# cdcseacave/openMVS

Measured on NVIDIA H100. Metric: Mpix/sec depth+normal (1920x1080, 9 neighbours), higher is better.
Workload: dtype f32

## Files before the change

### openmvs_b200/csrc/capi.cu

```cuda
#include "../../include/b200mvs.h"
#include "pm_common.cuh"
#include "sgm_front_sched.h"
#include <cuda.h>
#include <cmath>
#include <cstdio>
#include <cstring>
#include <string>
#include <vector>
#include <chrono>
#include <algorithm>
#include <cstdlib>

cudaError_t pm_configure_device();
cudaError_t pm_launch_score(const PMParams& P, bool geom, cudaStream_t s);
cudaError_t pm_launch_sweep(const PMParams& P, const void* tmapRef, bool geom, bool fourCtas, cudaStream_t s);
void pm_tma_box(int* w, int* h);
cudaError_t pm_launch_finalize(int n, float keep, const float4* plane, const float* cost, const uint32_t* bestViews,
	float* depth, float* normal, float* conf, uint32_t* viewsMap, cudaStream_t s);
cudaError_t pm_launch_pack(int n, const float* depth, const float* normal, float4* plane, cudaStream_t s);
cudaError_t pm_launch_unpack(int n, const float4* plane, float* depth, float* normal, cudaStream_t s);
struct SGMPixel { unsigned long long idx; short dmin, dmax; int pad; };
struct SGMParams {
	const float* lgray; const uchar3* lbgr; const float* rgray;
	int w, h, vw, vh;
	const SGMPixel* px;
	uint8_t* costs; uint16_t* accums;
	int P1;
	uint16_t P2s[256];
	int maxNumDisp;
};
cudaError_t sgm_configure_device();
cudaError_t sgm_launch_maxdisp(const SGMPixel* px, int n, unsigned long long numCosts, int* out8, cudaStream_t s);
cudaError_t sgm_launch_cost(const SGMParams& P, cudaStream_t s);
cudaError_t sgm_cost_tc_configure();
bool sgm_cost_tc_supports(int num);
cudaError_t sgm_cost_tc_launch(const SGMParams& P, int dmin, int num, cudaStream_t s);
cudaError_t sgm_launch_aggregate(const SGMParams& P, int dir, bool store, cudaStream_t s);
cudaError_t sgm_launch_aggregate_uniform(const SGMParams& P, int dir, int dmin, int num, bool ring, cudaStream_t s);
cudaError_t sgm_front_launch(const SGMParams& P, const FrontArgs& A, int blocks, int pd, cudaStream_t s);
int sgm_front_blocks_per_sm(int num, int pd);
bool sgm_front_supports(int num);
cudaError_t sgm_launch_wta(const SGMParams& P, int nVol, unsigned long long volStride, const uint16_t* more, int16_t* disparity, uint16_t* cost, cudaStream_t s);
cudaError_t sgm_launch_wta_uniform(const SGMParams& P, const uint16_t* second, int dmin, int num, int16_t* disparity, uint16_t* cost, cudaStream_t s);
int sgm_max_disparities();
cudaError_t sgm_launch_cross_check(int16_t* l2r, const int16_t* r2l, int w, int h, int th, cudaStream_t s);
cudaError_t sgm_launch_refine(const SGMPixel* px, const uint16_t* accums, int16_t* disparity, int n, int steps, cudaStream_t s);
#define FLT_MAX_NBR 16
struct FltView { const float* depth; const float* conf; int w, h; double fx, fy, cx, cy; double R[9], C[3]; };
// ... 224 lines not shown
	}
	return fn;
}

int prepare_ref_tmap(b200mvs_ctx* ctx, const DView& ref, cudaStream_t s) {
	ctx->tmapValid = false;
	EncodeTiledFn enc = ctx->dbg.noTMA ? nullptr : encode_tiled_fn();
	if (!enc) return B200MVS_OK;
	const float* base = ref.img; size_t pitchB = (size_t)ref.pitch*4;
	if (((uintptr_t)base & 15) || (pitchB & 15)) {
		pitchB = (((size_t)ref.w*4)+15)&~(size_t)15;
		CK(ctx->refPad.reserve(pitchB*ref.h));
		CK(cudaMemcpy2DAsync(ctx->refPad.p, pitchB, ref.img, (size_t)ref.pitch*4, (size_t)ref.w*4, ref.h, cudaMemcpyDeviceToDevice, s));
		base = ctx->refPad.as<float>();
	}
	int bw, bh; pm_tma_box(&bw, &bh);
	const cuuint64_t dims[2] = {(cuuint64_t)ref.w, (cuuint64_t)ref.h};
	const cuuint64_t strides[1] = {(cuuint64_t)pitchB};
	const cuuint32_t box[2] = {(cuuint32_t)bw, (cuuint32_t)bh};
	const cuuint32_t estr[2] = {1, 1};
	const CUresult r = enc(&ctx->tmapRef, CU_TENSOR_MAP_DATA_TYPE_FLOAT32, 2, (void*)base, dims, strides, box, estr,
		CU_TENSOR_MAP_INTERLEAVE_NONE, CU_TENSOR_MAP_SWIZZLE_NONE, CU_TENSOR_MAP_L2_PROMOTION_NONE, CU_TENSOR_MAP_FLOAT_OOB_FILL_NONE);
	ctx->tmapValid = (r == CUDA_SUCCESS);
	return B200MVS_OK;
}

int launch_sweep_timed(b200mvs_ctx* ctx, const PMParams& P, bool geom, cudaStream_t s) {
	if (ctx->timeSweeps) {
		while ((int)ctx->sweepEv.size() < 2*(ctx->nSweepEv+1)) {
			cudaEvent_t e; CK(cudaEventCreate(&e)); ctx->sweepEv.push_back(e);
		}
		CK(cudaEventRecord(ctx->sweepEv[2*ctx->nSweepEv], s));
	}
	CK(pm_launch_sweep(P, ctx->tmapValid ? &ctx->tmapRef : nullptr, geom, ctx->dbg.sweepFourCtas != 0, s)); ++ctx->launches;
	if (ctx->timeSweeps) {
		CK(cudaEventRecord(ctx->sweepEv[2*ctx->nSweepEv+1], s));
		++ctx->nSweepEv;
	}
	return B200MVS_OK;
}

int estimate_on_device(b200mvs_ctx* ctx, const DView* views, int nViews, float dMin, float dMax, int nGeometricIter,
	float* d_depth, float* d_normal, float* d_conf, uint32_t* d_views, cudaStream_t s)
{
	const b200mvs_params& o = ctx->prm;
	const int W = views[0].w, H = views[0].h;
	const bool geometric = nGeometricIter >= 0;
	int nSweepsPhoto, nRPhoto, nSweeps, nR;
	engine_schedule(o, false, nSweepsPhoto, nRPhoto);
	engine_schedule(o, geometric, nSweeps, nR);
	const int sweepBase = geometric ? nSweepsPhoto + nGeometricIter*nSweeps : 0;
	const int totalScale = !geometric ? std::max(0, o.nSubResolutionLevels) : 0;
	const size_t P0 = (size_t)W*H;
	if (ctx->mask && (ctx->maskW != W || ctx->maskH != H))
		return fail(ctx, B200MVS_ERR_ARG, "ignore-mask size differs from the reference image");
	CK(ctx->plane.reserve(P0*sizeof(float4)));
	CK(ctx->cost.reserve(P0*sizeof(float)));
	CK(ctx->best.reserve(P0*sizeof(uint32_t)));
	if (totalScale > 0) {
		CK(ctx->prior.reserve(P0*sizeof(float)));
		CK(ctx->lowPlane.reserve((size_t)(W/2+2)*(H/2+2)*sizeof(float4)));
		if (ctx->mask) CK(ctx->maskLevel.reserve((size_t)(W/2+2)*(H/2+2)));
		if ((int)ctx->pyr.size() < nViews) ctx->pyr.resize(nViews);
		for (int i = 0; i < nViews; ++i) {
			const size_t dw = (size_t)cvRoundI(views[i].w*0.5), dh = (size_t)cvRoundI(views[i].h*0.5);
			CK(ctx->pyr[i].reserve(dw*dh*sizeof(float)*(views[i].dmap ? 2 : 1)));
		}
// ... 472 lines not shown
	for (int i = 0; i < nViews; ++i)
		to_dview(views[i], views[i].image, views[i].stride_bytes ? views[i].stride_bytes/4 : views[i].width,
			views[i].depth, views[i].dstride_bytes ? views[i].dstride_bytes/4 : views[i].dwidth, dv[i]);
	{ const int rc2 = prepare_ref_tmap(ctx, dv[0], s); if (rc2) return rc2; }
	build_params(ctx->prm, dv.data(), nViews, dMin, dMax, lowres, (float4*)plane4, cost, nullptr, P, geom);
	P.tma = ctx->tmapValid ? 1 : 0;
	return B200MVS_OK;
}
int b200mvs_pm_score(b200mvs_ctx* ctx, const b200mvs_view* views, int nViews, float dMin, float dMax,
	const float* lowres, float* plane4, float* cost, void* stream)
{
	PMParams P; bool geom;
	if (!ctx) return B200MVS_ERR_ARG;
	CK(cudaSetDevice(ctx->device));
	cudaStream_t s = stream ? (cudaStream_t)stream : ctx->stream;
	int rc = block_params(ctx, views, nViews, dMin, dMax, lowres, plane4, cost, s, P, geom);
	if (rc) return rc;
	CK(pm_launch_score(P, geom, s));
	return B200MVS_OK;
}
int b200mvs_pm_sweep(b200mvs_ctx* ctx, const b200mvs_view* views, int nViews, float dMin, float dMax,
	const float* lowres, int sweep, int half, int nRandomIters, float* plane4, float* cost, void* stream)
{
	PMParams P; bool geom;
	if (!ctx) return B200MVS_ERR_ARG;
	CK(cudaSetDevice(ctx->device));
	cudaStream_t s = stream ? (cudaStream_t)stream : ctx->stream;
	int rc = block_params(ctx, views, nViews, dMin, dMax, lowres, plane4, cost, s, P, geom);
	if (rc) return rc;
	P.sweep = sweep; P.nRandomIters = nRandomIters;
	for (int colour = 0; colour < 2; ++colour) {
		if (half >= 0 && half != colour) continue;
		P.colour = colour;
		CK(pm_launch_sweep(P, ctx->tmapValid ? &ctx->tmapRef : nullptr, geom, ctx->dbg.sweepFourCtas != 0, s));
	}
	return B200MVS_OK;
}
int b200mvs_pm_finalize(b200mvs_ctx* ctx, int width, int height, float keep, const float* plane4, const float* cost,
	float* depth, float* normal, float* conf, void* stream)
{
	if (!ctx || !plane4 || !cost || !depth || !normal || !conf) return B200MVS_ERR_ARG;
	CK(cudaSetDevice(ctx->device));
	CK(pm_launch_finalize(width*height, keep, (const float4*)plane4, cost, nullptr, depth, normal, conf, nullptr,
		stream ? (cudaStream_t)stream : ctx->stream));
	return B200MVS_OK;
}

void b200mvs_sgm_default_params(b200mvs_sgm_params* p) { p->P1 = 3; p->P2 = 4; p->P2alpha = 14.f; p->P2beta = 38.f; }

int b200mvs_sgm_match_device(b200mvs_ctx* ctx, const float* leftGray, const uint8_t* leftBGR, const float* rightGray,
	int width, int height, const b200mvs_sgm_pixel* pixels, uint64_t numCosts, const b200mvs_sgm_params* prm,
	int stages, uint8_t* costs, uint16_t* accums, int16_t* disparity, uint16_t* cost, void* stream, b200mvs_stats* stats)
{
	if (!ctx) return B200MVS_ERR_ARG;
	if (!leftGray || !leftBGR || !rightGray || !pixels || width <= 6 || height <= 6 || numCosts == 0)
		return fail(ctx, B200MVS_ERR_ARG, "sgm: null image/pixel map or image too small");
	if ((stages & 4) && (!disparity || !cost))
		return fail(ctx, B200MVS_ERR_ARG, "sgm: null output map");
	b200mvs_sgm_params def; b200mvs_sgm_default_params(&def);
	if (!prm) prm = &def;
	CK(cudaSetDevice(ctx->device));
	cudaStream_t s = stream ? (cudaStream_t)stream : ctx->stream;
	static_assert(sizeof(b200mvs_sgm_pixel) == sizeof(SGMPixel), "pixel record layout");
	SGMParams P; memset(&P, 0, sizeof(P));
	P.lgray = leftGray; P.lbgr = (const uchar3*)leftBGR; P.rgray = rightGray;
	P.w = width; P.h = height; P.vw = width-6; P.vh = height-6;
	P.px = (const SGMPixel*)pixels;
// ... 446 lines not shown
```

### openmvs_b200/csrc/pm_kernels.cu

```cuda
#include "pm_common.cuh"
#include <math_constants.h>
#include <cstring>
#include <cuda.h>

namespace {

constexpr int BLOCK_X = 32;
constexpr int BLOCK_Y = 8;

constexpr int NTHREADS = BLOCK_X*BLOCK_Y;

struct PatchW {
	float2* s;
	float sumW, normSq0;
	__device__ __forceinline__ void set(int k, float a, float b) { s[k*NTHREADS] = make_float2(a, b); }
	__device__ __forceinline__ float2 get(int k) const { return s[k*NTHREADS]; }
};

constexpr int TILE_W = 2*BLOCK_X+2*PM_HALF;
constexpr int TILE_H = BLOCK_Y+2*PM_HALF;
constexpr int TILE_BYTES = TILE_W*TILE_H*4;

__device__ __forceinline__ uint32_t smem_u32(const void* p) { return (uint32_t)__cvta_generic_to_shared(p); }
__device__ __forceinline__ void mbar_init(uint64_t* bar, unsigned count) {
	asm volatile("mbarrier.init.shared::cta.b64 [%0], %1;" :: "r"(smem_u32(bar)), "r"(count) : "memory");
}
__device__ __forceinline__ void mbar_expect_tx(uint64_t* bar, unsigned bytes) {
	asm volatile("mbarrier.arrive.expect_tx.shared::cta.b64 _, [%0], %1;" :: "r"(smem_u32(bar)), "r"(bytes) : "memory");
}
__device__ __forceinline__ void mbar_wait(uint64_t* bar, unsigned parity) {
	asm volatile(
		"{\n"
		".reg .pred p;\n"
		"WAIT_LOOP:\n"
		"mbarrier.try_wait.parity.shared::cta.b64 p, [%0], %1;\n"
		"@p bra WAIT_DONE;\n"
		"bra WAIT_LOOP;\n"
		"WAIT_DONE:\n"
		"}\n" :: "r"(smem_u32(bar)), "r"(parity) : "memory");
}
__device__ __forceinline__ void tma_load_2d(void* dst, const CUtensorMap* map, int c0, int c1, uint64_t* bar) {
	asm volatile("cp.async.bulk.tensor.2d.shared::cluster.global.mbarrier::complete_tx::bytes [%0], [%1, {%2, %3}], [%4];"
		:: "r"(smem_u32(dst)), "l"(map), "r"(c0), "r"(c1), "r"(smem_u32(bar)) : "memory");
}

__device__ __forceinline__ void fill_patch_tile(const float* __restrict__ tile, int lx, int ly, PatchW& p) {
	const float sigmaColor = -1.f/(2.f*0.1f*0.1f);
	const float sigmaSpatial = -1.f/(2.f*9.f);
	const float center = tile[ly*TILE_W + lx];
	float acc = 0.f, sumW = 0.f;
	float w[PM_TEXELS], I[PM_TEXELS];
	#pragma unroll
	for (int i = 0; i < 5; ++i) {
		#pragma unroll
		for (int j = 0; j < 5; ++j) {
			const int dy = 2*i-PM_HALF, dx = 2*j-PM_HALF;
			const float v = tile[(ly+dy)*TILE_W + (lx+dx)];
			const float dI = v-center;
			const float wgt = expf(dI*dI*sigmaColor + float(dx*dx+dy*dy)*sigmaSpatial);
			w[i*5+j] = wgt;
			I[i*5+j] = v;
			acc += v*wgt;
			sumW += wgt;
		}
	}
	const float tm = acc/sumW;
	float nsq = 0.f;
	#pragma unroll
	for (int k = 0; k < PM_TEXELS; ++k) {
		const float t = I[k]-tm;
		const float tw = w[k]*t;
		nsq += tw*t;
		p.set(k, w[k], tw);
	}
	p.sumW = sumW;
	p.normSq0 = nsq;
}

__device__ __forceinline__ void fill_patch(const float* __restrict__ img, int pitch, int x, int y, PatchW& p) {
	const float sigmaColor = -1.f/(2.f*0.1f*0.1f);
	const float sigmaSpatial = -1.f/(2.f*9.f);
	const float center = __ldg(img + (size_t)y*pitch + x);
	float acc = 0.f, sumW = 0.f;
	float w[PM_TEXELS], I[PM_TEXELS];
	#pragma unroll
	for (int i = 0; i < 5; ++i) {
		#pragma unroll
		for (int j = 0; j < 5; ++j) {
			const int dy = 2*i-PM_HALF, dx = 2*j-PM_HALF;
			const float v = __ldg(img + (size_t)(y+dy)*pitch + (x+dx));
			const float dI = v-center;
			const float wgt = expf(dI*dI*sigmaColor + float(dx*dx+dy*dy)*sigmaSpatial);
			w[i*5+j] = wgt;
			I[i*5+j] = v;
			acc += v*wgt;
			sumW += wgt;
		}
	}
	const float tm = acc/sumW;
	float nsq = 0.f;
	#pragma unroll
	for (int k = 0; k < PM_TEXELS; ++k) {
		const float t = I[k]-tm;
		const float tw = w[k]*t;
		nsq += tw*t;
		p.set(k, w[k], tw);
	}
	p.sumW = sumW;
	p.normSq0 = nsq;
}

struct Hyp {
	float d;
	float3 n;
	float invd;
	float3 ms;
	float smooth;
};

struct Close {
	float d[4];
	float3 n[4];
	float rx[4], ry[4];
	unsigned mask;
};

__device__ __forceinline__ float fast_rcp(float x) { float r; asm("rcp.approx.ftz.f32 %0, %1;" : "=f"(r) : "f"(x)); return r; }
__device__ __forceinline__ float pow2neg(unsigned i) { return __int_as_float((int)(127u-i)<<23); }
__device__ __forceinline__ float dot3(const float3& a, const float3& b) { return a.x*b.x + a.y*b.y + a.z*b.z; }

__device__ __forceinline__ bool sample_depth_masked(const float* __restrict__ img, int pitch, float px, float py, float ref, float& v) {
	const int lx = (int)px, ly = (int)py;
	const float x = px-lx, x1 = 1.f-x, y = py-ly, y1 = 1.f-y;
	const float* r0 = img + (size_t)ly*pitch + lx;
	const float x0y0 = __ldg(r0), x1y0 = __ldg(r0+1), x0y1 = __ldg(r0+pitch), x1y1 = __ldg(r0+pitch+1);
	const bool b00 = fabsf(ref-x0y0)/ref < 0.03f, b10 = fabsf(ref-x1y0)/ref < 0.03f;
	const bool b01 = fabsf(ref-x0y1)/ref < 0.03f, b11 = fabsf(ref-x1y1)/ref < 0.03f;
	if (!b00 && !b10 && !b01 && !b11)
		return false;
	v = y1*(x1*(b00 ? x0y0 : (b10 ? x1y0 : (b01 ? x0y1 : x1y1))) + x*(b10 ? x1y0 : (b00 ? x0y0 : (b11 ? x1y1 : x0y1)))) +
	    y *(x1*(b01 ? x0y1 : (b11 ? x1y1 : (b00 ? x0y0 : x1y0))) + x*(b11 ? x1y1 : (b01 ? x0y1 : (b10 ? x1y0 : x0y0))));
	return true;
}

__device__ __forceinline__ void fetch_texels(const void* __restrict__ tex, int pitch, int lx, int ly,
	float& v00, float& v10, float& v01, float& v11)
{
	unsigned long long addr;
	const unsigned idx = (unsigned)(ly*pitch + lx);
	asm("mad.wide.u32 %0, %1, %2, %3;" : "=l"(addr) : "r"(idx), "r"(4u), "l"((unsigned long long)tex));
	const float* r0 = (const float*)addr;
	const float* r1 = r0+pitch;
	asm("ld.global.nc.L1::evict_last.f32 %0, [%1];" : "=f"(v00) : "l"(r0));
	asm("ld.global.nc.L1::evict_last.f32 %0, [%1+4];" : "=f"(v10) : "l"(r0));
	asm("ld.global.nc.L1::evict_last.f32 %0, [%1];" : "=f"(v01) : "l"(r1));
	asm("ld.global.nc.L1::evict_last.f32 %0, [%1+4];" : "=f"(v11) : "l"(r1));
}

template <bool GEOM>
__device__ __forceinline__ float score_view(const PMParams& P, const PMView& V, const PatchW& pt,
	float fx, float fy, float X0x, float X0y, const Hyp& h, float priorF, float priorD)
{
	float c0x = fmaf(V.Hm[0], h.ms.x, V.A[0]), c0y = fmaf(V.Hm[1], h.ms.x, V.A[3]), c0z = fmaf(V.Hm[2], h.ms.x, V.A[6]);
	float c1x = fmaf(V.Hm[0], h.ms.y, V.A[1]), c1y = fmaf(V.Hm[1], h.ms.y, V.A[4]), c1z = fmaf(V.Hm[2], h.ms.y, V.A[7]);
	const float xc = fmaf(V.Hm[0], h.invd, fmaf(V.A[0], fx, fmaf(V.A[1], fy, V.A[2])));
	const float yc = fmaf(V.Hm[1], h.invd, fmaf(V.A[3], fx, fmaf(V.A[4], fy, V.A[5])));
	const float zc = fmaf(V.Hm[2], h.invd, fmaf(V.A[6], fx, fmaf(V.A[7], fy, V.A[8])));
	float bx = fmaf(-4.f, c0x+c1x, xc), by = fmaf(-4.f, c0y+c1y, yc), bz = fmaf(-4.f, c0z+c1z, zc);
	c0x *= 2.f; c0y *= 2.f; c0z *= 2.f; c1x *= 2.f; c1y *= 2.f; c1z *= 2.f;
	const float xmax = float(V.w-2), ymax = float(V.h-2);
	bool ok;
	{
		const float x1 = fmaf(4.f, c0x, bx), y1 = fmaf(4.f, c0y, by), z1 = fmaf(4.f, c0z, bz);
		const float x2 = fmaf(4.f, c1x, bx), y2 = fmaf(4.f, c1y, by), z2 = fmaf(4.f, c1z, bz);
		const float x3 = fmaf(4.f, c1x, x1), y3 = fmaf(4.f, c1y, y1), z3 = fmaf(4.f, c1z, z1);
		const float zmin = fminf(fminf(bz, z1), fminf(z2, z3)), zmax = fmaxf(fmaxf(bz, z1), fmaxf(z2, z3));
		const float i0 = fast_rcp(bz), i1 = fast_rcp(z1), i2 = fast_rcp(z2), i3 = fast_rcp(z3);
		const float pxmin = fminf(fminf(bx*i0, x1*i1), fminf(x2*i2, x3*i3)), pxmax = fmaxf(fmaxf(bx*i0, x1*i1), fmaxf(x2*i2, x3*i3));
		const float pymin = fminf(fminf(by*i0, y1*i1), fminf(y2*i2, y3*i3)), pymax = fmaxf(fmaxf(by*i0, y1*i1), fmaxf(y2*i2, y3*i3));
		ok = (zmin > 0.f || zmax < 0.f) && pxmin >= 1.f && pymin >= 1.f && pxmax <= xmax && pymax <= ymax;
		ok = ok && (bx*i0 == bx*i0) && (x1*i1 == x1*i1) && (x2*i2 == x2*i2) && (x3*i3 == x3*i3)
		        && (by*i0 == by*i0) && (y1*i1 == y1*i1) && (y2*i2 == y2*i2) && (y3*i3 == y3*i3);
	}
	if (!__any_sync(__activemask(), ok))
		return P.thRobust;
	if (!ok) { bx = by = bz = 1.f; c0x = c0y = c0z = c1x = c1y = c1z = 0.f; }
	const void* tex = V.img;
	int pitch = V.pitch;
	asm volatile("" : "+r"(pitch), "+l"(tex));
	float sum = 0.f, sumSq = 0.f, num = 0.f;
	#pragma unroll
	for (int i = 0; i < 5; ++i) {
		float X = bx, Y = by, Z = bz;
		#pragma unroll
		for (int j = 0; j < 5; ++j) {
			const float iz = fast_rcp(Z);
			const float px = X*iz, py = Y*iz;
			const int lx = __float2int_rz(px), ly = __float2int_rz(py);
			const float ax = px-(float)lx, ay = py-(float)ly;
			float v00, v10, v01, v11;
			fetch_texels(tex, pitch, lx, ly, v00, v10, v01, v11);
			const float top = fmaf(ax, v10-v00, v00), bot = fmaf(ax, v11-v01, v01);
			const float v = fmaf(ay, bot-top, top);
			const float2 wk = pt.get(i*5+j);
			const float vw = v*wk.x;
			sum += vw; sumSq = fmaf(v, vw, sumSq); num = fmaf(v, wk.y, num);
			X += c0x; Y += c0y; Z += c0z;
		}
		bx += c1x; by += c1y; bz += c1z;
	}
	const bool bad = !ok;
	if (bad)
		return P.thRobust;
	const float normSq1 = sumSq - sum*sum/pt.sumW;
	const float nrmSq = pt.normSq0*normSq1;
	if (nrmSq <= 1e-16f)
		return P.thRobust;
	const float ncc = fminf(fmaxf(num/sqrtf(nrmSq), -1.f), 1.f);
	float score = (1.f-ncc)*h.smooth;
	if (GEOM) {
		if (V.dmap) {
			float consistency = 4.f;
			const float Xx = X0x*h.d, Xy = X0y*h.d, Xz = h.d;
			const float X1x = V.Tl[0]*Xx + V.Tl[1]*Xy + V.Tl[2]*Xz + V.Tm[0];
			const float X1y = V.Tl[3]*Xx + V.Tl[4]*Xy + V.Tl[5]*Xz + V.Tm[1];
			const float X1z = V.Tl[6]*Xx + V.Tl[7]*Xy + V.Tl[8]*Xz + V.Tm[2];
			if (X1z > 0.f) {
				const float x1x = X1x/X1z, x1y = X1y/X1z;
				if (x1x >= 1.f && x1y >= 1.f && x1x <= float(V.dw-2) && x1y <= float(V.dh-2)) {
					float depth1;
					if (sample_depth_masked(V.dmap, V.dpitch, x1x, x1y, X1z, depth1)) {
						const float Px = x1x*depth1, Py = x1y*depth1, Pz = depth1;
						const float Bx = V.Tr[0]*Px + V.Tr[1]*Py + V.Tr[2]*Pz + V.Tn[0];
						const float By = V.Tr[3]*Px + V.Tr[4]*Py + V.Tr[5]*Pz + V.Tn[1];
// ... 4 lines not shown
					}
				}
			}
			score += P.geomWeight*consistency;
		}
	}
	if (priorD > 0.f) {
		const float deltaDepth = fminf(fabsf(priorD-h.d)/priorD, 0.5f);
		score = (1.f-priorF)*score + priorF*deltaDepth;
	}
	return fminf(2.f, score);
}

template <bool GEOM>
__device__ __forceinline__ float score_pixel(const PMParams& P, const PatchW& pt,
	float fx, float fy, float X0x, float X0y, const Hyp& h, float priorF, float priorD, uint32_t& best)
{
	float s0 = CUDART_INF_F, s1 = CUDART_INF_F;
	int i0 = 255, i1 = 255;
	#pragma unroll 1
	for (int v = 0; v < P.nViews; ++v) {
		const float s = score_view<GEOM>(P, P.views[v], pt, fx, fy, X0x, X0y, h, priorF, priorD);
		if (s < s0) { s1 = s0; i1 = i0; s0 = s; i0 = v; }
		else if (s < s1) { s1 = s; i1 = v; }
	}
	if (P.nViews <= 1 || s1 >= P.thRobust) {
		best = 0xFFFFFF00u | (uint32_t)i0;
		return s0;
	}
	best = 0xFFFF0000u | ((uint32_t)i1<<8) | (uint32_t)i0;
	return (s0+s1)*0.5f;
}

__device__ __forceinline__ void make_hyp(const PMParams& P, float X0x, float X0y, float d, const float3& n,
	const Close& cl, bool useClose, Hyp& h)
{
	h.d = d; h.n = n;
	h.invd = 1.f/d;
	const float nX0 = n.x*X0x + n.y*X0y + n.z;
	const float s = 1.f/(nX0*d);
	h.ms = make_float3(n.x*P.ifx*s, (n.x*P.sk + n.y*P.ify)*s, (n.x*P.ox + n.y*P.oy + n.z)*s);
	float smooth = 1.f;
	if (useClose) {
		const float planeD = -d*nX0;
		const float nn = dot3(n, n);
		#pragma unroll
		for (int k = 0; k < 4; ++k) {
			if (cl.mask & (1u<<k)) {
				const float dist = (n.x*cl.rx[k] + n.y*cl.ry[k] + n.z)*cl.d[k] + planeD;
				const float rd = dist/d;
				const float factorDepth = expf(rd*rd*P.smoothSigmaDepth);
				float ca = dot3(n, cl.n[k])/sqrtf(nn*dot3(cl.n[k], cl.n[k]));
				ca = fminf(fmaxf(ca, -1.f), 1.f);
				const float ang = acosf(ca);
				const float factorNormal = expf(ang*ang*P.smoothSigmaNormal);
				smooth *= (1.f-P.smoothBonusDepth*factorDepth)*(1.f-P.smoothBonusNormal*factorNormal);
			}
		}
	}
	h.smooth = smooth;
}

__device__ __forceinline__ float3 dir2normal(float a, float b) {
	float sa, ca, sb, cb;
	sincosf(a, &sa, &ca);
	sincosf(b, &sb, &cb);
	return make_float3(ca*sb, sa*sb, cb);
}
__device__ __forceinline__ float3 random_normal(float u1, float u2, float X0x, float X0y) {
	const float kPI = 3.14159265358979323846f;
	const float a = 0.f + (kPI-0.f)*u1;
	const float b = 0.5f*kPI + (kPI-0.5f*kPI)*u2;
	float3 n = dir2normal(a, b);
	if (n.x*X0x + n.y*X0y + n.z > 0.f)
		n = make_float3(-n.x, -n.y, -n.z);
	return n;
}
__device__ __forceinline__ void correct_normal(float3& n, float X0x, float X0y) {
	const float cosAngLen = n.x*X0x + n.y*X0y + n.z;
	if (cosAngLen >= 0.f) {
		const float kPI = 3.14159265358979323846f;
		const float vlen = sqrtf(X0x*X0x + X0y*X0y + 1.f);
		const float ang = fminf((acosf(cosAngLen/vlen) - 0.5f*kPI)*1.01f, -0.001f);
		float3 w = make_float3(n.y*1.f - n.z*X0y, n.z*X0x - n.x*1.f, n.x*X0y - n.y*X0x);
		const float inv = 1.f/sqrtf(dot3(w, w));
// ... 22 lines not shown
	const bool inside = x >= PM_HALF && y >= PM_HALF && x < P.W-PM_HALF && y < P.H-PM_HALF;
	PatchW pt;
	pt.s = smemW + threadIdx.y*BLOCK_X + threadIdx.x;
	float priorD = 0.f, priorF = 0.f;
	bool ok = inside && !(P.mask && P.mask[(size_t)y*P.maskPitch + x] == 0);
	if (ok) {
		fill_patch(P.img0, P.pitch0, x, y, pt);
		if (P.lowres)
			priorD = fmaxf(__ldg(P.lowres + idx), 0.f);
		if (pt.normSq0 < P.thMagnitudeSq && !(priorD > 0.f))
			ok = false;
	}
	if (!ok) {
		P.plane[idx] = make_float4(0.f, 0.f, 0.f, 0.f);
		P.cost[idx] = 2.f;
		if (P.bestViews) P.bestViews[idx] = 0xFFFFFFFFu;
		return;
	}
	if (priorD > 0.f)
		priorF = expf(pt.normSq0*(-1.f/0.02f));
	const float fx = float(x), fy = float(y);
	const float X0x = fx*P.ifx + fy*P.sk + P.ox, X0y = fy*P.ify + P.oy;
	float4 pl = P.plane[idx];
	float3 n = make_float3(pl.x, pl.y, pl.z);
	float d = pl.w;
	const uint4 r = philox4x32_10(make_uint4((uint32_t)idx, 0u, 0u, 0u), make_uint2(P.seed, 0xB200C0DEu));
	if (!(P.dMin <= d && d < P.dMax)) {
		const float s = P.dMinSqr + (P.dMaxSqr-P.dMinSqr)*u32_to_unit(r.x);
		d = s*s;
		n = random_normal(u32_to_unit(r.y), u32_to_unit(r.z), X0x, X0y);
	} else if (n.x*X0x + n.y*X0y + n.z >= 0.f) {
		n = random_normal(u32_to_unit(r.x), u32_to_unit(r.y), X0x, X0y);
	}
	Close cl; cl.mask = 0;
	Hyp h;
	make_hyp(P, X0x, X0y, d, n, cl, false, h);
	uint32_t best;
	const float c = score_pixel<GEOM>(P, pt, fx, fy, X0x, X0y, h, priorF, priorD, best);
	P.plane[idx] = make_float4(n.x, n.y, n.z, d);
	P.cost[idx] = c;
	if (P.bestViews) P.bestViews[idx] = best;
}

template <bool GEOM, int MINB>
__global__ void __launch_bounds__(BLOCK_X*BLOCK_Y, MINB)
pm_sweep_kernel(const __grid_constant__ PMParams P, const __grid_constant__ CUtensorMap tmapRef)
{
	extern __shared__ __align__(128) unsigned char smemRaw[];
	float2* smemW = (float2*)smemRaw;
	float* tile = (float*)(smemRaw + PM_TEXELS*NTHREADS*sizeof(float2));
	uint64_t* bar = (uint64_t*)(tile + TILE_W*TILE_H);
	const int tid = threadIdx.y*BLOCK_X + threadIdx.x;
	if (P.tma) {
		if (tid == 0) {
			mbar_init(bar, 1);
			asm volatile("fence.proxy.async.shared::cta;" ::: "memory");
		}
		__syncthreads();
		if (tid == 0) {
			mbar_expect_tx(bar, TILE_BYTES);
			tma_load_2d(tile, &tmapRef, (int)blockIdx.x*(2*BLOCK_X)-PM_HALF, (int)blockIdx.y*BLOCK_Y-PM_HALF, bar);
		}
		mbar_wait(bar, 0);
	}
	const int y = blockIdx.y*BLOCK_Y + threadIdx.y;
	const int x = blockIdx.x*(2*BLOCK_X) + 2*threadIdx.x + ((y+P.colour)&1);
	if (x < PM_HALF || y < PM_HALF || x >= P.W-PM_HALF || y >= P.H-PM_HALF)
		return;
	if (P.mask && P.mask[(size_t)y*P.maskPitch + x] == 0)
		return;
	const int W = P.W, H = P.H;
	const size_t idx = (size_t)y*W + x;
	PatchW pt;
	pt.s = smemW + tid;
	if (P.tma)
		fill_patch_tile(tile, 2*(int)threadIdx.x + ((y+P.colour)&1) + PM_HALF, (int)threadIdx.y + PM_HALF, pt);
	else
		fill_patch(P.img0, P.pitch0, x, y, pt);
	float priorD = 0.f, priorF = 0.f;
	if (P.lowres)
		priorD = fmaxf(__ldg(P.lowres + idx), 0.f);
	if (pt.normSq0 < P.thMagnitudeSq && !(priorD > 0.f))
		return;
	if (priorD > 0.f)
		priorF = expf(pt.normSq0*(-1.f/0.02f));
	const float fx = float(x), fy = float(y);
	const float X0x = fx*P.ifx + fy*P.sk + P.ox, X0y = fy*P.ify + P.oy;

	const int dir = P.sweep & 1;
	const int nProp = P.propagation, farRings = P.farRings;
	Close cl; cl.mask = 0;
	unsigned todo = 0;
	unsigned farSel = 0;
	#pragma unroll
	for (int k = 0; k < 4; ++k) {
		const int kk = dir ? (k^2) : k;
		const int ox = (kk == 0) ? -1 : (kk == 2) ? 1 : 0;
		const int oy = (kk == 1) ? -1 : (kk == 3) ? 1 : 0;
		const bool ok = (kk == 0) ? (x > PM_HALF) : (kk == 1) ? (y > PM_HALF) : (kk == 2) ? (x < W-PM_HALF) : (y < H-PM_HALF);
		cl.d[k] = 0.f; cl.n[k] = make_float3(0.f, 0.f, 0.f); cl.rx[k] = 0.f; cl.ry[k] = 0.f;
		if (ok) {
			const size_t nidx = (size_t)(y+oy)*W + (x+ox);
			const float4 np = P.plane[nidx];
			const float nc = P.cost[nidx];
			bool changed = !cost_unchanged(nc);
			float bestC = 3.f;
			if (np.w > 0.f) {
				cl.mask |= 1u<<k;
				cl.d[k] = np.w; cl.n[k] = make_float3(np.x, np.y, np.z);
				const float nfx = float(x+ox), nfy = float(y+oy);
				cl.rx[k] = nfx*P.ifx + nfy*P.sk + P.ox; cl.ry[k] = nfy*P.ify + P.oy;
				bestC = fabsf(nc);
			}
			if (k < nProp) {
				unsigned ring = 0;
				for (int f = 1; f <= farRings; ++f) {
					const int qx = x+ox*(2*f+1), qy = y+oy*(2*f+1);
					if (qx < PM_HALF || qy < PM_HALF || qx >= W-PM_HALF || qy >= H-PM_HALF)
						break;
					const float fc = P.cost[(size_t)qy*W + qx];
					changed = changed || !cost_unchanged(fc);
					if (fabsf(fc) < bestC) { bestC = fabsf(fc); ring = (unsigned)f; }
				}
				if (bestC < P.keep && (changed || !P.skipUnchanged)) {
					todo |= 1u<<k;
					farSel |= ring<<(2*k);
				}
			}
		}
	}
	const float4 pl = P.plane[idx];
	float conf = fabsf(P.cost[idx]);
	float depth = pl.w;
	float3 normal = make_float3(pl.x, pl.y, pl.z);
	uint32_t bestViews = P.bestViews ? P.bestViews[idx] : 0xFFFFFFFFu;

	const int nR = P.nRandomIters;
	const int nRl = P.evalCap > 0 ? min(nR, max(P.evalCap-__popc(todo), 1)) : nR;
	const uint2 key = make_uint2(P.seed, 0xB200C0DEu);
	const uint32_t phase = 1u + (uint32_t)P.sweep;
	int mode = 0;
	bool entered = false;
	bool useClose = true;
	unsigned idxScale = 0;
	float scaleRange = 1.f, depthRange = 0.f, pa = 0.f, pb = 0.f;
	int nRestart = 0, nRefine = 0;
	#pragma unroll 1
	for (;;) {
		bool have = false, isRefine = false, alive = false, uc = true;
		float hd = 0.f, na = 0.f, nb = 0.f; float3 hn = make_float3(0.f, 0.f, 1.f);
		if (todo != 0u) {
			const int k = __ffs((int)todo)-1;
			todo &= todo-1u;
			const int kk = dir ? (k^2) : k;
			const int dist = 2*(int)((farSel>>(2*k))&3u)+1;
			const int qx = x + ((kk == 0) ? -dist : (kk == 2) ? dist : 0);
			const int qy = y + ((kk == 1) ? -dist : (kk == 3) ? dist : 0);
			const float4 qp = P.plane[(size_t)qy*W + qx];
			const bool vertical = (kk & 1) != 0;
			const float ncomp = vertical ? qp.y : qp.x;
			const float nx1 = vertical ? X0y : fmaf(fx, P.ifx, P.ox0);
			const float x1 = vertical ? fmaf(float(qy), P.ify, P.oy) : fmaf(float(qx), P.ifx, P.ox0);
			const float denom = qp.z + nx1*ncomp;
			hd = qp.w;
			if (!(fabsf(denom) < 0.0001f)) {
				const float dn = qp.w*(qp.z + x1*ncomp)/denom;
				if (P.dMin <= dn && dn < P.dMax)
// ... 16 lines not shown
					pa = atan2f(normal.y, normal.x);
					pb = acosf(normal.z);
				}
			}
			if (mode == 1 && nRestart >= nRl) mode = 3;
			alive = (mode == 1) || (mode == 2 && nRefine < nRl);
			uc = useClose;
			if (mode == 1) {
				const uint4 r = philox4x32_10(make_uint4((uint32_t)idx, phase, (uint32_t)nRestart, 0u), key);
				++nRestart;
				const float s = P.dMinSqr + (P.dMaxSqr-P.dMinSqr)*u32_to_unit(r.x);
				hd = s*s;
				hn = random_normal(u32_to_unit(r.y), u32_to_unit(r.z), X0x, X0y);
				have = true;
			} else if (mode == 2 && nRefine < nRl) {
				const uint4 r = philox4x32_10(make_uint4((uint32_t)idx, phase, (uint32_t)(nR+nRefine), 0u), key);
				++nRefine;
				hd = depth + depthRange*scaleRange*(2.f*u32_to_unit(r.x)-1.f);
				if (P.dMin <= hd && hd < P.dMax) {
					na = pa + P.angle1Range*scaleRange*(2.f*u32_to_unit(r.y)-1.f);
					nb = pb + P.angle2Range*scaleRange*(2.f*u32_to_unit(r.z)-1.f);
					hn = dir2normal(na, nb);
					have = hn.x*X0x + hn.y*X0y + hn.z < 0.f;
					isRefine = true;
				}
			}
		}
		if (!__any_sync(__activemask(), alive))
			break;
		if (!__any_sync(__activemask(), have))
			continue;
		if (have) {
			Hyp h;
			make_hyp(P, X0x, X0y, hd, hn, cl, uc, h);
			uint32_t bv;
			const float nconf = score_pixel<GEOM>(P, pt, fx, fy, X0x, X0y, h, priorF, priorD, bv);
			if (conf > nconf) {
				conf = nconf; depth = hd; normal = hn; bestViews = bv;
				if (isRefine) {
					pa = na; pb = nb;
					++idxScale;
					scaleRange = pow2neg(idxScale);
				}
			}
		}
	}
	const bool same = depth == pl.w && normal.x == pl.x && normal.y == pl.y && normal.z == pl.z;
	P.plane[idx] = make_float4(normal.x, normal.y, normal.z, depth);
	P.cost[idx] = (same && P.skipUnchanged) ? -conf : conf;
	if (P.bestViews) P.bestViews[idx] = bestViews;
}

__global__ void pm_finalize_kernel(int n, float keep, const float4* __restrict__ plane, const float* __restrict__ cost,
	const uint32_t* __restrict__ bestViews, float* __restrict__ depth, float* __restrict__ normal, float* __restrict__ conf,
	uint32_t* __restrict__ viewsMap)
{
	const int i = blockIdx.x*blockDim.x + threadIdx.x;
	if (i >= n) return;
	const float4 p = plane[i];
	const float c = fabsf(cost[i]);
	float d = p.w, cf; float3 nn = make_float3(p.x, p.y, p.z);
	uint32_t bv = bestViews ? bestViews[i] : 0xFFFFFFFFu;
	if (d <= 0.f || c >= keep) {
		d = 0.f; cf = 0.f; nn = make_float3(0.f, 0.f, 0.f); bv = 0xFFFFFFFFu;
	} else {
		cf = c >= 1.f ? 0.f : 1.f-c;
		const uint32_t a = bv & 0xFFu, b = (bv>>8) & 0xFFu;
		bv = 0xFFFF0000u | (max(a, b)<<8) | min(a, b);
	}
	depth[i] = d; conf[i] = cf;
	normal[3*(size_t)i] = nn.x; normal[3*(size_t)i+1] = nn.y; normal[3*(size_t)i+2] = nn.z;
	if (viewsMap) viewsMap[i] = bv;
}

__global__ void pm_pack_kernel(int n, const float* __restrict__ depth, const float* __restrict__ normal, float4* __restrict__ plane) {
	const int i = blockIdx.x*blockDim.x + threadIdx.x;
	if (i >= n) return;
	plane[i] = make_float4(normal[3*(size_t)i], normal[3*(size_t)i+1], normal[3*(size_t)i+2], depth[i]);
}
__global__ void pm_unpack_kernel(int n, const float4* __restrict__ plane, float* __restrict__ depth, float* __restrict__ normal) {
	const int i = blockIdx.x*blockDim.x + threadIdx.x;
	if (i >= n) return;
	const float4 p = plane[i];
	depth[i] = p.w;
	normal[3*(size_t)i] = p.x; normal[3*(size_t)i+1] = p.y; normal[3*(size_t)i+2] = p.z;
}

constexpr size_t W_BYTES = (size_t)PM_TEXELS*NTHREADS*sizeof(float2);
constexpr size_t SWEEP_SMEM = W_BYTES + TILE_BYTES + 16;

template <bool GEOM>
cudaError_t configure_one() {
	cudaError_t e = cudaFuncSetAttribute(pm_sweep_kernel<GEOM, 3>, cudaFuncAttributeMaxDynamicSharedMemorySize, (int)SWEEP_SMEM);
	if (e != cudaSuccess) return e;
	e = cudaFuncSetAttribute(pm_sweep_kernel<GEOM, 4>, cudaFuncAttributeMaxDynamicSharedMemorySize, (int)SWEEP_SMEM);
	if (e != cudaSuccess) return e;
	return cudaFuncSetAttribute(pm_score_kernel<GEOM>, cudaFuncAttributeMaxDynamicSharedMemorySize, (int)W_BYTES);
}

}

cudaError_t pm_configure_device() {
	cudaError_t e;
	if ((e = configure_one<false>()) != cudaSuccess) return e;
	return configure_one<true>();
}
cudaError_t pm_launch_score(const PMParams& P, bool geom, cudaStream_t s) {
	dim3 block(BLOCK_X, BLOCK_Y), grid((P.W+BLOCK_X-1)/BLOCK_X, (P.H+BLOCK_Y-1)/BLOCK_Y);
	if (geom) pm_score_kernel<true><<<grid, block, W_BYTES, s>>>(P); else pm_score_kernel<false><<<grid, block, W_BYTES, s>>>(P);
	return cudaGetLastError();
}
template <int MINB>
static void launch_sweep(const PMParams& P, const CUtensorMap& map, bool geom, dim3 grid, dim3 block, cudaStream_t s) {
	if (geom) pm_sweep_kernel<true, MINB><<<grid, block, SWEEP_SMEM, s>>>(P, map); else pm_sweep_kernel<false, MINB><<<grid, block, SWEEP_SMEM, s>>>(P, map);
}
cudaError_t pm_launch_sweep(const PMParams& P, const void* tmapRef, bool geom, bool fourCtas, cudaStream_t s) {
	dim3 block(BLOCK_X, BLOCK_Y), grid((P.W+2*BLOCK_X-1)/(2*BLOCK_X), (P.H+BLOCK_Y-1)/BLOCK_Y);
	CUtensorMap map; memset(&map, 0, sizeof(map));
	if (tmapRef) memcpy(&map, tmapRef, sizeof(map));
	if (fourCtas) launch_sweep<4>(P, map, geom, grid, block, s);
	else launch_sweep<3>(P, map, geom, grid, block, s);
	return cudaGetLastError();
}
void pm_tma_box(int* w, int* h) { *w = TILE_W; *h = TILE_H; }
cudaError_t pm_launch_finalize(int n, float keep, const float4* plane, const float* cost, const uint32_t* bestViews,
	float* depth, float* normal, float* conf, uint32_t* viewsMap, cudaStream_t s) {
	pm_finalize_kernel<<<(n+255)/256, 256, 0, s>>>(n, keep, plane, cost, bestViews, depth, normal, conf, viewsMap);
	return cudaGetLastError();
}
cudaError_t pm_launch_pack(int n, const float* depth, const float* normal, float4* plane, cudaStream_t s) {
	pm_pack_kernel<<<(n+255)/256, 256, 0, s>>>(n, depth, normal, plane);
	return cudaGetLastError();
}
cudaError_t pm_launch_unpack(int n, const float4* plane, float* depth, float* normal, cudaStream_t s) {
	pm_unpack_kernel<<<(n+255)/256, 256, 0, s>>>(n, plane, depth, normal);
	return cudaGetLastError();
}
```

Baseline: 26.41.

## Alias TMA tile with patch weights and recompute neighbour planes to cut registers

The reference tile now shares shared memory with the patch-weight buffer, using a barrier between reading the tile and writing the weights, so each block needs less shared memory. The per-thread Close struct is removed and neighbour planes are reloaded from global memory inside make_hyp, which lowers register pressure. Bilinear tap addressing now floors with a magic-number float add instead of float-to-int conversion. The four-CTA launch-bounds variant and the debug option that selected it are removed. The reloads add global traffic, and inactive threads now have to reach the barrier before they return.

```diff
diff --git a/openmvs_b200/csrc/capi.cu b/openmvs_b200/csrc/capi.cu
--- a/openmvs_b200/csrc/capi.cu
+++ b/openmvs_b200/csrc/capi.cu
@@ -13,7 +13,7 @@
 
 cudaError_t pm_configure_device();
 cudaError_t pm_launch_score(const PMParams& P, bool geom, cudaStream_t s);
-cudaError_t pm_launch_sweep(const PMParams& P, const void* tmapRef, bool geom, bool fourCtas, cudaStream_t s);
+cudaError_t pm_launch_sweep(const PMParams& P, const void* tmapRef, bool geom, cudaStream_t s);
 void pm_tma_box(int* w, int* h);
 cudaError_t pm_launch_finalize(int n, float keep, const float4* plane, const float* cost, const uint32_t* bestViews,
 	float* depth, float* normal, float* conf, uint32_t* viewsMap, cudaStream_t s);
@@ -304,7 +304,7 @@
 		}
 		CK(cudaEventRecord(ctx->sweepEv[2*ctx->nSweepEv], s));
 	}
-	CK(pm_launch_sweep(P, ctx->tmapValid ? &ctx->tmapRef : nullptr, geom, ctx->dbg.sweepFourCtas != 0, s)); ++ctx->launches;
+	CK(pm_launch_sweep(P, ctx->tmapValid ? &ctx->tmapRef : nullptr, geom, s)); ++ctx->launches;
 	if (ctx->timeSweeps) {
 		CK(cudaEventRecord(ctx->sweepEv[2*ctx->nSweepEv+1], s));
 		++ctx->nSweepEv;
@@ -843,7 +843,7 @@
 	for (int colour = 0; colour < 2; ++colour) {
 		if (half >= 0 && half != colour) continue;
 		P.colour = colour;
-		CK(pm_launch_sweep(P, ctx->tmapValid ? &ctx->tmapRef : nullptr, geom, ctx->dbg.sweepFourCtas != 0, s));
+		CK(pm_launch_sweep(P, ctx->tmapValid ? &ctx->tmapRef : nullptr, geom, s));
 	}
 	return B200MVS_OK;
 }
diff --git a/openmvs_b200/csrc/pm_kernels.cu b/openmvs_b200/csrc/pm_kernels.cu
--- a/openmvs_b200/csrc/pm_kernels.cu
+++ b/openmvs_b200/csrc/pm_kernels.cu
@@ -44,7 +44,7 @@
 		:: "r"(smem_u32(dst)), "l"(map), "r"(c0), "r"(c1), "r"(smem_u32(bar)) : "memory");
 }
 
-__device__ __forceinline__ void fill_patch_tile(const float* __restrict__ tile, int lx, int ly, PatchW& p) {
+__device__ __forceinline__ void fill_patch_tile(const float* tile, int lx, int ly, PatchW& p) {
 	const float sigmaColor = -1.f/(2.f*0.1f*0.1f);
 	const float sigmaSpatial = -1.f/(2.f*9.f);
 	const float center = tile[ly*TILE_W + lx];
@@ -65,14 +65,17 @@
 		}
 	}
 	const float tm = acc/sumW;
-	float nsq = 0.f;
+	float nsq = 0.f, tw[PM_TEXELS];
 	#pragma unroll
 	for (int k = 0; k < PM_TEXELS; ++k) {
 		const float t = I[k]-tm;
-		const float tw = w[k]*t;
-		nsq += tw*t;
-		p.set(k, w[k], tw);
-	}
+		tw[k] = w[k]*t;
+		nsq += tw[k]*t;
+	}
+	__syncthreads();
+	#pragma unroll
+	for (int k = 0; k < PM_TEXELS; ++k)
+		p.set(k, w[k], tw[k]);
 	p.sumW = sumW;
 	p.normSq0 = nsq;
 }
@@ -118,13 +121,6 @@
 	float smooth;
 };
 
-struct Close {
-	float d[4];
-	float3 n[4];
-	float rx[4], ry[4];
-	unsigned mask;
-};
-
 __device__ __forceinline__ float fast_rcp(float x) { float r; asm("rcp.approx.ftz.f32 %0, %1;" : "=f"(r) : "f"(x)); return r; }
 __device__ __forceinline__ float pow2neg(unsigned i) { return __int_as_float((int)(127u-i)<<23); }
 __device__ __forceinline__ float dot3(const float3& a, const float3& b) { return a.x*b.x + a.y*b.y + a.z*b.z; }
@@ -143,12 +139,20 @@
 	return true;
 }
 
-__device__ __forceinline__ void fetch_texels(const void* __restrict__ tex, int pitch, int lx, int ly,
+constexpr unsigned TAP_BIAS = 0x4B000000u;
+__device__ __forceinline__ float tap_floor(float p, unsigned& bits) {
+	const float t = __fadd_rz(p, 0x1p23f);
+	bits = __float_as_uint(t);
+	return t - 0x1p23f;
+}
+
+__device__ __forceinline__ unsigned long long tap_base(const float* img) { return (unsigned long long)img - 4ull*TAP_BIAS; }
+__device__ __forceinline__ void fetch_texels(unsigned long long base, int pitch, unsigned xb, unsigned yb,
 	float& v00, float& v10, float& v01, float& v11)
 {
 	unsigned long long addr;
-	const unsigned idx = (unsigned)(ly*pitch + lx);
-	asm("mad.wide.u32 %0, %1, %2, %3;" : "=l"(addr) : "r"(idx), "r"(4u), "l"((unsigned long long)tex));
+	const unsigned idx = (yb-TAP_BIAS)*(unsigned)pitch + xb;
+	asm("mad.wide.u32 %0, %1, %2, %3;" : "=l"(addr) : "r"(idx), "r"(4u), "l"(base));
 	const float* r0 = (const float*)addr;
 	const float* r1 = r0+pitch;
 	asm("ld.global.nc.L1::evict_last.f32 %0, [%1];" : "=f"(v00) : "l"(r0));
@@ -185,9 +189,9 @@
 	if (!__any_sync(__activemask(), ok))
 		return P.thRobust;
 	if (!ok) { bx = by = bz = 1.f; c0x = c0y = c0z = c1x = c1y = c1z = 0.f; }
-	const void* tex = V.img;
+	unsigned long long base = tap_base(V.img);
 	int pitch = V.pitch;
-	asm volatile("" : "+r"(pitch), "+l"(tex));
+	asm volatile("" : "+r"(pitch), "+l"(base));
 	float sum = 0.f, sumSq = 0.f, num = 0.f;
 	#pragma unroll
 	for (int i = 0; i < 5; ++i) {
@@ -196,10 +200,10 @@
 		for (int j = 0; j < 5; ++j) {
 			const float iz = fast_rcp(Z);
 			const float px = X*iz, py = Y*iz;
-			const int lx = __float2int_rz(px), ly = __float2int_rz(py);
-			const float ax = px-(float)lx, ay = py-(float)ly;
+			unsigned xb, yb;
+			const float ax = px-tap_floor(px, xb), ay = py-tap_floor(py, yb);
 			float v00, v10, v01, v11;
-			fetch_texels(tex, pitch, lx, ly, v00, v10, v01, v11);
+			fetch_texels(base, pitch, xb, yb, v00, v10, v01, v11);
 			const float top = fmaf(ax, v10-v00, v00), bot = fmaf(ax, v11-v01, v01);
 			const float v = fmaf(ay, bot-top, top);
 			const float2 wk = pt.get(i*5+j);
@@ -270,8 +274,14 @@
 	return (s0+s1)*0.5f;
 }
 
-__device__ __forceinline__ void make_hyp(const PMParams& P, float X0x, float X0y, float d, const float3& n,
-	const Close& cl, bool useClose, Hyp& h)
+__device__ __forceinline__ void close_offset(int dir, int k, int& ox, int& oy) {
+	const int kk = dir ? (k^2) : k;
+	ox = (kk == 0) ? -1 : (kk == 2) ? 1 : 0;
+	oy = (kk == 1) ? -1 : (kk == 3) ? 1 : 0;
+}
+
+__device__ __forceinline__ void make_hyp(const PMParams& P, int x, int y, float X0x, float X0y, float d, const float3& n,
+	int dir, unsigned closeMask, Hyp& h)
 {
 	h.d = d; h.n = n;
 	h.invd = 1.f/d;
@@ -279,16 +289,23 @@
 	const float s = 1.f/(nX0*d);
 	h.ms = make_float3(n.x*P.ifx*s, (n.x*P.sk + n.y*P.ify)*s, (n.x*P.ox + n.y*P.oy + n.z)*s);
 	float smooth = 1.f;
-	if (useClose) {
+	if (closeMask != 0u) {
+		asm volatile("" : "+r"(x), "+r"(y));
 		const float planeD = -d*nX0;
 		const float nn = dot3(n, n);
 		#pragma unroll
 		for (int k = 0; k < 4; ++k) {
-			if (cl.mask & (1u<<k)) {
-				const float dist = (n.x*cl.rx[k] + n.y*cl.ry[k] + n.z)*cl.d[k] + planeD;
+			if (closeMask & (1u<<k)) {
+				int ox, oy;
+				close_offset(dir, k, ox, oy);
+				const float4 np = P.plane[(size_t)(y+oy)*P.W + (x+ox)];
+				const float3 cn = make_float3(np.x, np.y, np.z);
+				const float nfx = float(x+ox), nfy = float(y+oy);
+				const float rx = nfx*P.ifx + nfy*P.sk + P.ox, ry = nfy*P.ify + P.oy;
+				const float dist = (n.x*rx + n.y*ry + n.z)*np.w + planeD;
 				const float rd = dist/d;
 				const float factorDepth = expf(rd*rd*P.smoothSigmaDepth);
-				float ca = dot3(n, cl.n[k])/sqrtf(nn*dot3(cl.n[k], cl.n[k]));
+				float ca = dot3(n, cn)/sqrtf(nn*dot3(cn, cn));
 				ca = fminf(fmaxf(ca, -1.f), 1.f);
 				const float ang = acosf(ca);
 				const float factorNormal = expf(ang*ang*P.smoothSigmaNormal);
@@ -377,9 +394,8 @@
 	} else if (n.x*X0x + n.y*X0y + n.z >= 0.f) {
 		n = random_normal(u32_to_unit(r.x), u32_to_unit(r.y), X0x, X0y);
 	}
-	Close cl; cl.mask = 0;
 	Hyp h;
-	make_hyp(P, X0x, X0y, d, n, cl, false, h);
+	make_hyp(P, x, y, X0x, X0y, d, n, 0, 0u, h);
 	uint32_t best;
 	const float c = score_pixel<GEOM>(P, pt, fx, fy, X0x, X0y, h, priorF, priorD, best);
 	P.plane[idx] = make_float4(n.x, n.y, n.z, d);
@@ -387,14 +403,14 @@
 	if (P.bestViews) P.bestViews[idx] = best;
 }
 
-template <bool GEOM, int MINB>
-__global__ void __launch_bounds__(BLOCK_X*BLOCK_Y, MINB)
+template <bool GEOM>
+__global__ void __launch_bounds__(BLOCK_X*BLOCK_Y, 3)
 pm_sweep_kernel(const __grid_constant__ PMParams P, const __grid_constant__ CUtensorMap tmapRef)
 {
 	extern __shared__ __align__(128) unsigned char smemRaw[];
 	float2* smemW = (float2*)smemRaw;
-	float* tile = (float*)(smemRaw + PM_TEXELS*NTHREADS*sizeof(float2));
-	uint64_t* bar = (uint64_t*)(tile + TILE_W*TILE_H);
+	float* tile = (float*)smemRaw;
+	uint64_t* bar = (uint64_t*)(smemRaw + PM_TEXELS*NTHREADS*sizeof(float2));
 	const int tid = threadIdx.y*BLOCK_X + threadIdx.x;
 	if (P.tma) {
 		if (tid == 0) {
@@ -410,18 +426,21 @@
 	}
 	const int y = blockIdx.y*BLOCK_Y + threadIdx.y;
 	const int x = blockIdx.x*(2*BLOCK_X) + 2*threadIdx.x + ((y+P.colour)&1);
-	if (x < PM_HALF || y < PM_HALF || x >= P.W-PM_HALF || y >= P.H-PM_HALF)
-		return;
-	if (P.mask && P.mask[(size_t)y*P.maskPitch + x] == 0)
-		return;
+	const bool active = x >= PM_HALF && y >= PM_HALF && x < P.W-PM_HALF && y < P.H-PM_HALF
+		&& !(P.mask && P.mask[(size_t)y*P.maskPitch + x] == 0);
 	const int W = P.W, H = P.H;
 	const size_t idx = (size_t)y*W + x;
 	PatchW pt;
 	pt.s = smemW + tid;
-	if (P.tma)
+	if (P.tma) {
 		fill_patch_tile(tile, 2*(int)threadIdx.x + ((y+P.colour)&1) + PM_HALF, (int)threadIdx.y + PM_HALF, pt);
-	else
+		if (!active)
+			return;
+	} else {
+		if (!active)
+			return;
 		fill_patch(P.img0, P.pitch0, x, y, pt);
+	}
 	float priorD = 0.f, priorF = 0.f;
 	if (P.lowres)
 		priorD = fmaxf(__ldg(P.lowres + idx), 0.f);
@@ -434,16 +453,15 @@
 
 	const int dir = P.sweep & 1;
 	const int nProp = P.propagation, farRings = P.farRings;
-	Close cl; cl.mask = 0;
+	unsigned closeMask = 0;
 	unsigned todo = 0;
 	unsigned farSel = 0;
 	#pragma unroll
 	for (int k = 0; k < 4; ++k) {
 		const int kk = dir ? (k^2) : k;
-		const int ox = (kk == 0) ? -1 : (kk == 2) ? 1 : 0;
-		const int oy = (kk == 1) ? -1 : (kk == 3) ? 1 : 0;
+		int ox, oy;
+		close_offset(dir, k, ox, oy);
 		const bool ok = (kk == 0) ? (x > PM_HALF) : (kk == 1) ? (y > PM_HALF) : (kk == 2) ? (x < W-PM_HALF) : (y < H-PM_HALF);
-		cl.d[k] = 0.f; cl.n[k] = make_float3(0.f, 0.f, 0.f); cl.rx[k] = 0.f; cl.ry[k] = 0.f;
 		if (ok) {
 			const size_t nidx = (size_t)(y+oy)*W + (x+ox);
 			const float4 np = P.plane[nidx];
@@ -451,10 +469,7 @@
 			bool changed = !cost_unchanged(nc);
 			float bestC = 3.f;
 			if (np.w > 0.f) {
-				cl.mask |= 1u<<k;
-				cl.d[k] = np.w; cl.n[k] = make_float3(np.x, np.y, np.z);
-				const float nfx = float(x+ox), nfy = float(y+oy);
-				cl.rx[k] = nfx*P.ifx + nfy*P.sk + P.ox; cl.ry[k] = nfy*P.ify + P.oy;
+				closeMask |= 1u<<k;
 				bestC = fabsf(nc);
 			}
 			if (k < nProp) {
@@ -474,10 +489,12 @@
 			}
 		}
 	}
-	const float4 pl = P.plane[idx];
-	float conf = fabsf(P.cost[idx]);
-	float depth = pl.w;
-	float3 normal = make_float3(pl.x, pl.y, pl.z);
+	float depth, conf = fabsf(P.cost[idx]);
+	float3 normal;
+	{
+		const float4 pl = P.plane[idx];
+		depth = pl.w; normal = make_float3(pl.x, pl.y, pl.z);
+	}
 	uint32_t bestViews = P.bestViews ? P.bestViews[idx] : 0xFFFFFFFFu;
 
 	const int nR = P.nRandomIters;
@@ -560,7 +577,7 @@
 			continue;
 		if (have) {
 			Hyp h;
-			make_hyp(P, X0x, X0y, hd, hn, cl, uc, h);
+			make_hyp(P, x, y, X0x, X0y, hd, hn, dir, uc ? closeMask : 0u, h);
 			uint32_t bv;
 			const float nconf = score_pixel<GEOM>(P, pt, fx, fy, X0x, X0y, h, priorF, priorD, bv);
 			if (conf > nconf) {
@@ -573,6 +590,7 @@
 			}
 		}
 	}
+	const float4 pl = P.plane[idx];
 	const bool same = depth == pl.w && normal.x == pl.x && normal.y == pl.y && normal.z == pl.z;
 	P.plane[idx] = make_float4(normal.x, normal.y, normal.z, depth);
 	P.cost[idx] = (same && P.skipUnchanged) ? -conf : conf;
@@ -615,13 +633,12 @@
 }
 
 constexpr size_t W_BYTES = (size_t)PM_TEXELS*NTHREADS*sizeof(float2);
-constexpr size_t SWEEP_SMEM = W_BYTES + TILE_BYTES + 16;
+constexpr size_t SWEEP_SMEM = W_BYTES + 16;
+static_assert(TILE_BYTES <= W_BYTES, "the reference tile must fit inside the patch weights");
 
 template <bool GEOM>
 cudaError_t configure_one() {
-	cudaError_t e = cudaFuncSetAttribute(pm_sweep_kernel<GEOM, 3>, cudaFuncAttributeMaxDynamicSharedMemorySize, (int)SWEEP_SMEM);
-	if (e != cudaSuccess) return e;
-	e = cudaFuncSetAttribute(pm_sweep_kernel<GEOM, 4>, cudaFuncAttributeMaxDynamicSharedMemorySize, (int)SWEEP_SMEM);
+	cudaError_t e = cudaFuncSetAttribute(pm_sweep_kernel<GEOM>, cudaFuncAttributeMaxDynamicSharedMemorySize, (int)SWEEP_SMEM);
 	if (e != cudaSuccess) return e;
 	return cudaFuncSetAttribute(pm_score_kernel<GEOM>, cudaFuncAttributeMaxDynamicSharedMemorySize, (int)W_BYTES);
 }
@@ -638,16 +655,11 @@
 	if (geom) pm_score_kernel<true><<<grid, block, W_BYTES, s>>>(P); else pm_score_kernel<false><<<grid, block, W_BYTES, s>>>(P);
 	return cudaGetLastError();
 }
-template <int MINB>
-static void launch_sweep(const PMParams& P, const CUtensorMap& map, bool geom, dim3 grid, dim3 block, cudaStream_t s) {
-	if (geom) pm_sweep_kernel<true, MINB><<<grid, block, SWEEP_SMEM, s>>>(P, map); else pm_sweep_kernel<false, MINB><<<grid, block, SWEEP_SMEM, s>>>(P, map);
-}
-cudaError_t pm_launch_sweep(const PMParams& P, const void* tmapRef, bool geom, bool fourCtas, cudaStream_t s) {
+cudaError_t pm_launch_sweep(const PMParams& P, const void* tmapRef, bool geom, cudaStream_t s) {
 	dim3 block(BLOCK_X, BLOCK_Y), grid((P.W+2*BLOCK_X-1)/(2*BLOCK_X), (P.H+BLOCK_Y-1)/BLOCK_Y);
 	CUtensorMap map; memset(&map, 0, sizeof(map));
 	if (tmapRef) memcpy(&map, tmapRef, sizeof(map));
-	if (fourCtas) launch_sweep<4>(P, map, geom, grid, block, s);
-	else launch_sweep<3>(P, map, geom, grid, block, s);
+	if (geom) pm_sweep_kernel<true><<<grid, block, SWEEP_SMEM, s>>>(P, map); else pm_sweep_kernel<false><<<grid, block, SWEEP_SMEM, s>>>(P, map);
 	return cudaGetLastError();
 }
 void pm_tma_box(int* w, int* h) { *w = TILE_W; *h = TILE_H; }
```

After: 28.50, median of 6. +7.9%, better.
